# abignoli/EdgeGraph3D

Measured on AMD Instinct MI355X. Metric: triangulated edge-points/sec, higher is better.
Workload: dtype f64

## Files before the change

### edgegraph3d_amd/api.py

```python
import ctypes as C
import os

import numpy as np

from . import _cdefs as D

_LIB = None


class Eg3dError(RuntimeError):
    pass


def lib_path():
    return os.environ.get("EG3D_LIB") or os.path.join(os.path.dirname(os.path.abspath(__file__)), "libeg3d.so")


def lib():
    global _LIB
    if _LIB is None:
        path = lib_path()
        if not os.path.exists(path):
            raise Eg3dError("libeg3d.so (HIP extension) is missing: run `python -m edgegraph3d_amd.build`. "
                            "There is no CPU fallback.")
# ... 159 lines not shown
        return None
    return C.c_void_p(x.ptr if isinstance(x, DeviceArray) else int(x))


class Context:
    def __init__(self, scene_ptr, device=0, _handle=None):
        self._h = C.c_void_p()
        if _handle is not None:
            self._h = _handle
        else:
            _check(lib().eg3d_create(scene_ptr, device, C.byref(self._h)), "eg3d_create")
        nv, dv = C.c_int32(), C.c_int32()
        _check(lib().eg3d_context_info(self._h, C.byref(nv), C.byref(dv)), "eg3d_context_info")
        self.n_views, self.device = nv.value, dv.value

    def clone(self):
        h = C.c_void_p()
        _check(lib().eg3d_clone(self._h, C.byref(h)), "eg3d_clone")
        return Context(None, _handle=h)

    def set_pipelining(self, lanes=0, units=0):
        _check(lib().eg3d_set_pipelining(self._h, lanes, units), "eg3d_set_pipelining")

    def close(self):
        if self._h:
            lib().eg3d_destroy(self._h)
            self._h = C.c_void_p()

    def __del__(self):
        try:
            self.close()
        except Exception:
            pass

    def grid(self, view, which):
        ncols, nrows = C.c_uint32(), C.c_uint32()
        off, ids = D.u32p(), D.u32p()
        _check(lib().eg3d_get_grid(self._h, view, which, C.byref(ncols), C.byref(nrows), C.byref(off), C.byref(ids)),
               "eg3d_get_grid")
        n = ncols.value * nrows.value
        o = D.as_np(off, n + 1, np.uint32)
        return ncols.value, nrows.value, o, D.as_np(ids, int(o[-1]), np.uint32)

    def upload_seeds(self, seeds_ptr):
        _check(lib().eg3d_upload_seeds(self._h, seeds_ptr), "eg3d_upload_seeds")

# ... 308 lines not shown
```

### edgegraph3d_amd/csrc/eg3d_api.hip

```cpp
#include <hip/hip_runtime.h>
#include <hipcub/hipcub.hpp>

#include <algorithm>
#include <cstdio>
#include <cstdlib>

#include <atomic>
#include <chrono>
#include <cmath>
#include <cstring>
#include <memory>
#include <mutex>
#include <string>
#include <thread>
#include <vector>

#include "../../include/eg3d_host.h"
#include "eg3d_api_internal.h"
#include "eg3d_host_copy.h"

thread_local std::string eg3d::api::g_err;
extern "C" const char* eg3d_last_error(void) { return g_err.c_str(); }

static std::atomic<int64_t> g_live_device_bytes{0};
// ... 948 lines not shown
extern "C" int eg3d_probe_hyp_sections(eg3d_ctx* c, double* sum, double* slowest, uint32_t* counts) {
  if (!c || !sum || !slowest || !counts) return EG3D_ERR_ARG;
  const uint32_t n = c->last_nhyp;
  std::vector<HypResult> r(n ? n : 1);
  if (n) HIP_TRY(hipMemcpy(r.data(), c->b_res.p, sizeof(HypResult) * n, hipMemcpyDeviceToHost));
  for (int k = 0; k < 6; k++) sum[k] = slowest[k] = 0;
  for (int k = 0; k < 5; k++) counts[k] = 0;
  counts[0] = n;
  for (uint32_t h = 0; h < n; h++) {
    if (r[h].status & HYP_TRI) counts[1]++;
    if (r[h].status & HYP_D1) counts[2]++;
    if (r[h].status & HYP_D2) counts[3]++;
    if (hyp_compatible(r[h].status, r[h].n1, r[h].n2)) counts[4]++;
    sum[0] += r[h].n1;
    sum[1] += r[h].n2;
    if (r[h].n1 > slowest[0]) slowest[0] = r[h].n1;
    if (r[h].n2 > slowest[1]) slowest[1] = r[h].n2;
    if (r[h].n1 + r[h].n2 >= 32) sum[2] += 1;
  }
  return EG3D_OK;
}

#endif
#if defined(EG3D_WITH_K3C_ENGINE) && (defined(EG3D_SECTION_TIMING) || defined(EG3D_K3C_TIMING))
namespace eg3d { int k3c_dbg_read(unsigned long long* out, int reset); }
extern "C" int eg3d_probe_k3c(unsigned long long* out128, int reset) { return eg3d::k3c_dbg_read(out128, reset); }
#endif
```

### edgegraph3d_amd/csrc/eg3d_api_internal.h

```cpp
#pragma once
#include <hip/hip_runtime.h>

#include <algorithm>
#include <chrono>
#include <cstdlib>
#include <cstring>
#include <initializer_list>
#include <memory>
#include <mutex>
#include <string>
#include <vector>

#include "../../include/eg3d.h"
#include "eg3d_kernels.h"
#include "eg3d_k8_replay.h"
#include "eg3d_k9_polymatch.h"
#include "eg3d_k10_simgraph.h"
#include "eg3d_k11_louvain.h"

#define EG3D_API_BEGIN namespace eg3d { namespace api __attribute__((visibility("hidden"))) {
#define EG3D_API_END }}

EG3D_API_BEGIN
extern thread_local std::string g_err;
// ... 146 lines not shown

using namespace eg3d;
using namespace eg3d::api;

struct eg3d_ctx {
  int device = 0;
  Tunables tune;
  hipStream_t stream = nullptr;
  int V = 0, W = 0, H = 0;
  DevScene ds;
  DevBuf b_camP, b_F, b_Fv, b_vpo, b_pvo, b_vtx, b_pls, b_ple, b_g30o, b_g30i, b_g4o, b_g4i, b_bbo, b_bb;
  std::shared_ptr<DevOwner> scene_owner;
  std::shared_ptr<HostGrids> hg;
  uint32_t gw[2] = {0, 0}, gh[2] = {0, 0};
  uint32_t grid_dropped = 0;
  uint32_t n_seeds = 0;
  std::shared_ptr<std::vector<uint32_t>> h_trk;
  DevBuf b_toff, b_tview, b_txy;
  std::shared_ptr<DevOwner> seeds_owner;
  WorkBuf b_sv_seed, b_map_view, b_map_entry, b_map_n, b_raw_cnt, b_raw_off, b_cand_pl, b_start_hits, b_cand_cnt,
      b_start_cnt, b_task_off, b_task_seed, b_task_entry, b_task_hit, b_task_k, b_task_list_off, b_list_cnt, b_list_ptr,
      b_hits, b_tasks, b_nhyp, b_hyp_off, b_res, b_arena, b_ctr, b_cs_task, b_valid, b_chain_off, b_chains,
      b_cscratch, b_couts, b_cpts, b_cobs, b_cpoff, b_cooff, b_scan_tmp, b_scanchk, b_cost, b_cidx, b_cost2, b_order, b_redo[2];
  WorkBuf o_X, o_off, o_view, o_pl, o_seg, o_xy, o_key;
  WorkBuf f_X, f_off, f_view, f_xy, f_Xo, f_inl;
  WorkBuf r_hist, r_blk, r_Xo, r_inl, c_X, c_off, c_view, c_pl, c_seg, c_xy, c_key;
  bool compact_nt = false;
  WorkBuf d_first, d_cnt, d_keep;
  bool dedup_valid = false;
  WorkBuf prim_tmp;
  WorkBuf k8_cnt, k8_slot, k8_last, k8_firstof, k8_flag, k8_rank, k8_lastof, k8_plid, k8_key[2], k8_val[2], k8_map, k8_sflag, k8_pos;
  WorkBuf g_nodeX, g_nodept, g_pls, g_ple, g_conoff, g_conpl, g_ivoff, g_ivss, g_ivsxy, g_ives, g_ivexy;
  WorkBuf k9_svseed, k9_cnt, k9_pl, k9_dist, k9_acc, k9_accoff, k9_first, k9_parent, k9_root, k9_ckey, k9_rank, k9_key[2], k9_ctr,
      k9_ref, k9_rowoff, k9_plids;
  WorkBuf k10_svseed, k10_cnt, k10_off, k10_pair[2], k10_crkey, k10_cpoff, k10_cpview, k10_cppl, k10_croff, k10_crpoint, k10_weight, k10_vis,
      k10_npairs, k10_pairoff, k10_nkey[2], k10_nodeof, k10_nodeg, k10_nodeview, k10_nodepl, k10_edge[2], k10_dkey[2], k10_dval[2],
      k10_adjoff, k10_adjnode, k10_ctr;
  WorkBuf k11[K11B_COUNT];
  uint32_t louvain_log2_slots = 0;
  uint64_t simgraph_pair_budget = 0;
  int replay_table_bits = 0;
  uint32_t n_pl = 0, n_vtx = 0;
  WorkBuf b_sets_off, b_sets_ids;
  WorkBuf b_fscratch, b_queue, b_items;
  WorkBuf b_pools, b_stage_pts, b_stage_obs, b_stage_used;
  uint32_t slots_per_xcd = 0;
// ... 125 lines not shown
```

### edgegraph3d_amd/csrc/eg3d_api_match.hip

```cpp
#include <sys/mman.h>

#include <atomic>
#include <condition_variable>
#include <cstdio>
#include <shared_mutex>
#include <thread>

#include "eg3d_api_internal.h"
#include "eg3d_host_copy.h"

#ifndef EG3D_D2H_CHUNK
#define EG3D_D2H_CHUNK ((size_t)16 << 20)
#endif
#define EG3D_D2H_CHUNK_SMALL ((size_t)2 << 20)
#define EG3D_D2H_BIG_CLOUD ((size_t)96 << 20)
#ifndef EG3D_D2H_RING
#define EG3D_D2H_RING 4
#endif
static int ensure_d2h_ring(eg3d_ctx* c, size_t cloud_bytes) {
  const size_t want = cloud_bytes >= EG3D_D2H_BIG_CLOUD ? EG3D_D2H_CHUNK : EG3D_D2H_CHUNK_SMALL;
  if (c->pinned && c->ring_chunk >= want) return EG3D_OK;
  if (c->pinned) (void)hipHostFree(c->pinned);
  c->pinned = nullptr;
  c->ring_chunk = c->pinned_cap = 0;
// ... 339 lines not shown
    const int ic = rb.add(c->b_ctr.p, sizeof(Counters) / 4);
    const int it = rb.add(c->b_chain_off.as<uint32_t>() + nt, 1);
    const int iw = rb.add(c->b_scanchk.as<uint32_t>(), 1);
    rb.clear_after(c->b_scanchk.as<uint32_t>());
    BUF_TRY(rb.run());
    memcpy(&hc, rb.item(ic), sizeof(Counters));
    if (c->tune.trace_arena)
      fprintf(stderr, "eg3d: hypothesis arena: %u hypotheses, %u points used of %u (%.2f per hypothesis)%s\n", B.n_hyp,
              hc.arena_used, arena_cap, B.n_hyp ? (double)hc.arena_used / B.n_hyp : 0.0,
              (hc.flags & CTR_ARENA_OVERFLOW) ? " OVERFLOW" : "");
    if (!(hc.flags & CTR_ARENA_OVERFLOW)) {
      if (*rb.item(iw)) return wrapped_error("chains");
      B.n_chains = *rb.item(it);
      break;
    }
    if (attempt >= 6) {
      g_err = "eg3d: hypothesis arena overflow";
      return EG3D_ERR_CAPACITY;
    }
    arena_cap = std::max<uint32_t>(arena_cap * 2, hc.arena_used + (hc.arena_used >> 2));
    if (B.n_hyp) c->arena_per_hyp = std::max(c->arena_per_hyp, 1.25 * (double)arena_cap / (double)B.n_hyp);
  }
  H.flags |= (hc.flags & 0xffu);
  BUF_TRY(c->b_chains.ensure(sizeof(ChainSeed) * (B.n_chains + 1)));
  launch_compact_chains(st, nt, c->b_cs_task.as<ChainSeed>(), c->b_valid.as<uint32_t>(), c->b_chain_off.as<uint32_t>(),
                        c->b_chains.as<ChainSeed>());
  HIP_TRY(hipEventRecord(c->eb[4], st));
  return EG3D_OK;
}

struct ExpandState {
  uint32_t c0 = 0, nc = 0;
  uint32_t redo_n = 0;
  int redo_buf = 0;
  uint64_t stage_lim_pts = ~0ull, stage_lim_obs = ~0ull;
  ChainLayout L{};
  bool engine = false;
  uint32_t eng_waves = 0, eng_lanes = 64;
  SlotPools pools{};
  StageBuf stage{};
  uint32_t n_launch = 0;
  const uint32_t* launch_order = nullptr;
  Counters hc{};
  uint32_t np = 0, no = 0;
  unsigned long long stage_used[2] = {0, 0};
  float ms_expand = 0, ms_emit = 0;
// ... 1146 lines not shown
```

### edgegraph3d_amd/csrc/eg3d_dev_geom.h

```cpp
#pragma once
#include <stdint.h>

#if defined(__HIPCC__)
#include <hip/hip_runtime.h>
#define EG3D_HD __host__ __device__ inline
#define EG3D_HD_FLAT __host__ __device__ inline __attribute__((always_inline))
#else
#define EG3D_HD inline
#define EG3D_HD_FLAT inline
#endif

#if defined(__HIP_DEVICE_COMPILE__)
#define EG3D_SQRTF(x) __builtin_sqrtf(x)
#define EG3D_SQRT(x) __dsqrt_rn(x)
#else
#include <math.h>
#define EG3D_SQRTF(x) sqrtf(x)
#define EG3D_SQRT(x) sqrt(x)
#endif

#ifndef EG3D_STAT
#define EG3D_STAT(i)
#endif

// ... 397 lines not shown
        got = true;
        seg_found = (uint32_t)(to_start ? first - k : first + k - 1);
        break;
      }
      W.shift(k);
    }
    if (!got) return WALK_EXTREME;
  }
  out.seg = seg_found;
  out.x = hx;
  out.y = hy;
  if (bounded) {
    float dsq = dist2(hx, hy, p.x, p.y);
    if (dsq < (min_d * min_d) || dsq > (max_d * max_d)) return WALK_BOUND;
  }
  return WALK_FOUND;
}
template <class VPtr>
EG3D_HD uint32_t walk_by_line_pf(const PlRefT<VPtr>& pl, const PlPt& p, uint32_t direction, float la, float lb, float lc,
                                 bool bounded, float min_d, float max_d, PlPt& out) {
  VtxWindow<VPtr> W;
  if (!walk_by_line_open(pl, p, direction, W)) return WALK_BAD_DIR;
  return walk_by_line_run(pl, p, direction, la, lb, lc, bounded, min_d, max_d, W, out);
}

EG3D_HD float polyline_closest(const PlRef& pl, float px, float py, PlPt& out) {
  float bx, by;
  float best = seg_closest(px, py, pl.v[0].x, pl.v[0].y, pl.v[1].x, pl.v[1].y, bx, by);
  uint32_t bseg = 0;
  for (uint32_t i = 2; i < pl.n; i++) {
    float cx, cy;
    float d = seg_closest(px, py, pl.v[i - 1].x, pl.v[i - 1].y, pl.v[i].x, pl.v[i].y, cx, cy);
    if (d < best) {
      best = d;
      bx = cx;
      by = cy;
      bseg = i - 1;
    }
  }
  out.seg = bseg;
  out.x = bx;
  out.y = by;
  return best;
}

EG3D_HD float polyline_closest_range(const PlRef& pl, float px, float py, uint32_t s0, uint32_t s1, PlPt& out) {
// ... 155 lines not shown
```

### edgegraph3d_amd/csrc/eg3d_k3a_engine.h

```cpp
#pragma once
#include "eg3d_dev_pipeline.h"

#include "eg3d_dev_coopgn.h"

namespace eg3d {

#ifdef EG3D_GN_COUNTERS
#define K3A_T0() unsigned long long kt_[3] = {0, 0, 0}, kc_[4] = {0, 0, 0, 0}, kt0_ = __builtin_readcyclecounter(), kt1_
#define K3A_T(i) (kt1_ = __builtin_readcyclecounter(), kt_[i] += kt1_ - kt0_, kt0_ = kt1_)
#define K3A_C(i, v) (kc_[i] += (v))
#define K3A_TEND(kern)                                                \
  if (lane == 0) {                                                    \
    for (int q_ = 0; q_ < 3; q_++) EG3D_GN_DBG(113 + 7 * (kern) + q_, kt_[q_]); \
    for (int q_ = 0; q_ < 4; q_++) EG3D_GN_DBG(116 + 7 * (kern) + q_, kc_[q_]); \
  }
#else
#define K3A_T0() ((void)0)
#define K3A_T(i) ((void)0)
#define K3A_C(i, v) ((void)0)
#define K3A_TEND(kern) ((void)0)
#endif

#define EG3D_K3A_STAGE EG3D_K3A_STAGE_POINTS
#ifndef EG3D_K3A_SPEC
// ... 42 lines not shown
    return r;
  }
};

__device__ __forceinline__ uint32_t k3a_slots_per_lane(uint32_t n_working) {
  uint32_t k = 64u / n_working, p = 1;
  while (p * 2 <= k && p * 2 <= (uint32_t)EG3D_K3A_SPEC) p *= 2;
  return p;
}

__device__ __forceinline__ void k3a_serve(K3aShared& sh, const DevScene& s, uint32_t lane) {
  __syncthreads();
  if (sh.reqM[lane] & 1u) {
    const Obs o[3] = {sh.req[lane][0], sh.req[lane][1], sh.req[lane][2]};
    float X[3] = {0.0f, 0.0f, 0.0f};
    uint32_t f = 0;
    const bool ok = triangulate3(s.cam_P, o, X, f);
    sh.resX[lane][0] = X[0];
    sh.resX[lane][1] = X[1];
    sh.resX[lane][2] = X[2];
    sh.resF[lane] = (ok ? 1u : 0u) | (f << 8);
  }
  __syncthreads();
}

__device__ __forceinline__ HPoint k3a_point_of_slot(const K3aShared& sh, uint32_t slot) {
  HPoint hp;
  hp.X[0] = sh.resX[slot][0];
  hp.X[1] = sh.resX[slot][1];
  hp.X[2] = sh.resX[slot][2];
  hp.nobs = 3;
  hp.o[0] = sh.req[slot][0];
  hp.o[1] = sh.req[slot][1];
  hp.o[2] = sh.req[slot][2];
  hp.pad = 0;
  return hp;
}

enum : uint32_t { K3A_IDLE = 0, K3A_GEN = 1, K3A_REQ = 2, K3A_END = 3 };
enum : uint32_t { K3A_TRI0 = 0, K3A_ORIENT = 1, K3A_REPLAY = 2, K3A_OPP = 3 };

__global__ void __launch_bounds__(64, EG3D_K3A_WAVES) k3a_orient(DevScene s, StageAView a, const TaskDesc* tasks,
                                                                 const uint32_t* hyp_off, uint32_t n_hyp, HypResult* res,
                                                                 uint32_t cap, HPoint* arena, uint32_t arena_cap,
                                                                 Counters* ctr, uint32_t* queue, uint32_t lanes_per_wave,
                                                                 uint32_t* items, uint32_t* n_items) {
// ... 37 lines not shown
  auto issue = [&](uint32_t slot, int q, uint32_t round_off) {
    const PlPt pA = L.get(0), pB = L.get(1 + (q >> 1)), pC = L.get(3 + (q & 1));
    Obs o;
    o.view = (uint32_t)view[0];
    o.pl = pl[0];
    o.seg = pA.seg;
    o.x = pA.x;
    o.y = pA.y;
    sh.req[slot][0] = o;
    o.view = (uint32_t)view[1];
    o.pl = pl[1];
    o.seg = pB.seg;
    o.x = pB.x;
    o.y = pB.y;
    sh.req[slot][1] = o;
    o.view = (uint32_t)view[2];
    o.pl = pl[2];
    o.seg = pC.seg;
    o.x = pC.x;
    o.y = pC.y;
    sh.req[slot][2] = o;
    sh.reqM[slot] = 1u | ((uint32_t)q << 8) | (round_off << 10);
  };
  K3A_T0();

  for (;;) {
    const unsigned long long working = __ballot(!(st == K3A_IDLE && exhausted));
    if (!working) break;
    K3A_C(0, 1);
    K3A_C(2, __popcll(working));
    const uint32_t K = k3a_slots_per_lane((uint32_t)__popcll(working));
    const uint32_t slot0 = (uint32_t)__popcll(working & lt) * K;
    sh.reqM[lane] = 0;
    __syncthreads();
    uint32_t n_issued = 0;
    if (st == K3A_END) {
      bool finish = false, to_d1 = false, restart = false;
      if (phase == K3A_TRI0) {
        if (okmask & 1u) {
          status |= HYP_TRI;
          e = 0;
          phase = K3A_ORIENT;
          restart = true;
        } else {
          finish = true;
        }
// ... 96 lines not shown
        const TaskDesc d = tasks[t_cur];
        Obs c[3];
        hypothesis_hits(a, d, t_cur, h - hyp_off[t_cur], c);
        for (int k = 0; k < 3; k++) {
          view[k] = (int32_t)c[k].view;
          pl[k] = c[k].pl;
          L.load_polyline(s, k, view[k], pl[k]);
        }
        to_hits(c);
        status = 0;
        flags = 0;
        n1 = n2 = 0;
        base = 0xffffffffu;
        arena_ok = false;
        for (int k = 0; k < 3; k++) d1[k] = d2[k] = 0;
        X0[0] = X0[1] = X0[2] = 0.0f;
        phase = K3A_TRI0;
        reqmask = 1u;
        okmask = 0;
        st = K3A_REQ;
      }
    }
    dead_round = 0xffffffffu;
    if (st == K3A_GEN) {
      uint32_t walkers = alive;
      for (uint32_t round_off = 0;; round_off++) {
        uint32_t fl = 0, m = walkers;
        const PlRef pa = L.polyline(s, 0);
        PlPt q;
        const uint32_t w = walk_by_distance_pf(pa, L.get(0), dirA, EG3D_FOLLOW_STEP, q);
        if (w & WALK_BAD_DIR) fl |= 8u;
        if (w & WALK_EXTREME) {
          m = 0;
        } else {
          L.set(0, q);
          float la = 0.0f, lb = 0.0f, lc = 0.0f;
          PlRef pk = pa;
#pragma unroll 1
          for (int idx = 0; idx < 4 && m; idx++) {
            const int k = 1 + (idx >> 1), j = idx & 1;
            const uint32_t users = k == 1 ? (3u << (2 * j)) : (5u << j);
            if (j == 0) {
              if (!epiline(s.F, s.F_valid, s.n_views, view[0], view[k], q.x, q.y, la, lb, lc)) {
                m = 0;
                break;
              }
              pk = L.polyline(s, k);
            }
            if (!(m & users)) continue;
            PlPt r;
            const uint32_t wr = walk_by_line_pf(pk, L.get(2 * k - 1 + j), k == 1 ? dirB[j] : dirC[j], la, lb, lc, false, 0.0f,
                                                0.0f, r);
            if (wr & WALK_BAD_DIR) fl |= 8u;
            if (wr & WALK_FOUND)
              L.set(2 * k - 1 + j, r);
            else
              m &= ~users;
          }
        }
        if (phase != K3A_REPLAY) flags |= fl;
        if (round_off == 0) {
          reqmask = m;
          okmask = 0;
          if (!m) {
            if (phase == K3A_REPLAY) n1 = i_rep;
            if (phase == K3A_ORIENT) {
              alive = 0;
              rounds++;
            }
            st = K3A_END;
            break;
          }
          st = K3A_REQ;
          while (reqmask && n_issued < K) {
            const int qq = __ffs((int)reqmask) - 1;
            reqmask &= reqmask - 1u;
            issue(slot0 + n_issued, qq, 0u);
            n_issued++;
          }
          if (reqmask) break;
        } else {
          if (!m) {
            if (phase == K3A_REPLAY)
              n1 = i_rep + round_off;
            else
              dead_round = round_off;
            break;
          }
          uint32_t mm = m;
          while (mm) {
            const int qq = __ffs((int)mm) - 1;
            mm &= mm - 1u;
            issue(slot0 + n_issued, qq, round_off);
            n_issued++;
          }
        }
        const uint32_t cm = (uint32_t)__popc(m);
        bool more;
        if (phase == K3A_REPLAY)
          more = i_rep + round_off + 1u < n1 && n_issued < K;
        else if (phase == K3A_ORIENT)
          more = cm >= 2u && n_issued + cm <= K && round_off < 14u;
        else
          more = false;
        if (!more) break;
        walkers = m;
      }
    }
    if (st == K3A_REQ && n_issued == 0) {
      while (reqmask && n_issued < K) {
        const int qq = __ffs((int)reqmask) - 1;
        reqmask &= reqmask - 1u;
        issue(slot0 + n_issued, qq, 0u);
        n_issued++;
      }
    }
    K3A_T(0);
    K3A_C(1, __popcll(__ballot(sh.reqM[lane] & 1u)));
    k3a_serve(sh, s, lane);
    K3A_T(1);
    if (n_issued) {
      if (phase == K3A_REPLAY) {
        for (uint32_t j = 0; j < n_issued; j++)
          if (arena_ok) arena[base + i_rep + j] = k3a_point_of_slot(sh, slot0 + j);
        i_rep += n_issued;
        st = K3A_END;
      } else if (phase == K3A_ORIENT) {
        uint32_t cur = 0;
        bool decided = false;
// ... 28 lines not shown
          }
          st = K3A_END;
        }
      } else {
        const uint32_t f = sh.resF[slot0];
        flags |= f >> 8;
        if (f & 1u) {
          okmask |= 1u;
          if (phase == K3A_TRI0) {
            X0[0] = sh.resX[slot0][0];
            X0[1] = sh.resX[slot0][1];
            X0[2] = sh.resX[slot0][2];
          } else {
            status |= HYP_D2;
            n2 = 1;
            if (arena_ok) arena[base + n1] = k3a_point_of_slot(sh, slot0);
          }
        }
        st = K3A_END;
      }
    }
    K3A_T(2);
  }
  K3A_TEND(0);
}

template <class T>
__device__ __forceinline__ T k3a_pick(const T a[3], int i) {
  return i == 0 ? a[0] : i == 1 ? a[1] : a[2];
}
__device__ __forceinline__ bool k3a_follow_request(const DevScene& s, const K3aLane& L, const int32_t view3[3],
                                                   int st_start, const uint32_t dirs[3], const int32_t ids[3],
                                                   int& st_used, PlPt sel_pt[3], uint32_t& fl) {
#pragma unroll 1
  for (int st = st_start; st < 3; st++) {
    const int32_t sv = k3a_pick(view3, st);
    const int sd = (sv == ids[0]) ? 0 : (sv == ids[1]) ? 1 : 2;
    const PlRef ps = L.polyline(s, sd);
    PlPt q;
    const uint32_t w = walk_by_distance_pf(ps, L.get(3 + st), k3a_pick(dirs, sd), EG3D_FOLLOW_STEP, q);
    if (w & WALK_BAD_DIR) fl |= 8u;
    if (w & WALK_EXTREME) continue;
    int found = 0;
    PlPt r1 = q, r2 = q;
#pragma unroll 1
    for (int t = 0; t < 2; t++) {
      const int i = t == 0 ? (st == 0 ? 1 : 0) : (st == 2 ? 1 : 2);
      const int32_t cv = k3a_pick(view3, i);
      float la, lb, lc;
      if (!epiline(s.F, s.F_valid, s.n_views, sv, cv, q.x, q.y, la, lb, lc)) continue;
      const int cd = (cv == ids[0]) ? 0 : (cv == ids[1]) ? 1 : 2;
      const PlRef pk = L.polyline(s, cd);
      PlPt r;
      const uint32_t wr =
          walk_by_line_pf(pk, L.get(3 + i), k3a_pick(dirs, cd), la, lb, lc, true, EG3D_FOLLOW_MIN, EG3D_FOLLOW_MAX, r);
      if (wr & WALK_BAD_DIR) fl |= 8u;
      if (wr & WALK_FOUND) {
        found++;
        if (t == 0)
          r1 = r;
        else
          r2 = r;
      }
    }
    if (found < 2) continue;
    st_used = st;
    sel_pt[0] = q;
    sel_pt[1] = r1;
    sel_pt[2] = r2;
    return true;
  }
  return false;
}

__global__ void __launch_bounds__(64, EG3D_K3A_WAVES) k3a_follow_spec(DevScene s, HypResult* res, HPoint* scratch,
                                                                      uint32_t cap, HPoint* arena, uint32_t arena_cap,
                                                                      Counters* ctr, uint32_t* queue, uint32_t lanes_per_wave,
                                                                      const uint32_t* items, const uint32_t* n_items_p) {
  __shared__ K3aShared sh;
  const uint32_t lane = threadIdx.x;
  const K3aLane L{&sh, lane};
  const unsigned long long lt = (1ull << lane) - 1ull;
  const uint32_t stage = cap < (uint32_t)EG3D_K3A_STAGE ? cap : (uint32_t)EG3D_K3A_STAGE;
  HPoint* scr = scratch + ((size_t)blockIdx.x * 64 + lane) * stage;
  uint32_t big_base = 0xffffffffu;
  const uint32_t n_items = *n_items_p;
  bool have = false, exhausted = lane >= lanes_per_wave;
  uint32_t h = 0, dir = 0, n_init = 0, n_new = 0, init_off = 0, flags = 0;
  int st_start = 0;
  uint32_t dirs[3] = {0, 0, 0};
  int32_t ids[3] = {0, 0, 0};
  int32_t cview[3] = {0, 0, 0};
  uint32_t cpl[3] = {0, 0, 0};
  K3A_T0();
  for (;;) {
    while (!have && !exhausted) {
      const uint32_t i = atomicAdd(queue, 1u);
      if (i >= n_items) {
        exhausted = true;
        break;
      }
      const uint32_t item = items[i];
      h = item >> 1;
      dir = item & 1u;
      const HypResult& r = res[h];
      const uint32_t stt = r.status;
      if (!(dir == 0 ? (stt & HYP_D1) : (stt & HYP_D2))) continue;
      n_init = dir == 0 ? r.n1 : r.n2;
      init_off = dir == 0 ? r.pts1_off : r.pts2_off;
      if (n_init == 0 || init_off == 0xffffffffu) continue;
      for (int k = 0; k < 3; k++) dirs[k] = dir == 0 ? r.dirs1[k] : r.dirs2[k];
      const HPoint last = arena[init_off + n_init - 1];
      for (int k = 0; k < 3; k++) {
        cview[k] = (int32_t)last.o[k].view;
        cpl[k] = last.o[k].pl;
        ids[k] = cview[k];
        L.load_polyline(s, k, cview[k], cpl[k]);
        PlPt p;
        p.seg = last.o[k].seg;
        p.x = last.o[k].x;
        p.y = last.o[k].y;
        L.set(k, p);
      }
      n_new = 0;
      flags = 0;
      st_start = 0;
      big_base = 0xffffffffu;
      have = true;
    }
    const unsigned long long working = __ballot(have);
    if (!working) break;
    const uint32_t K = k3a_slots_per_lane((uint32_t)__popcll(working));
    const uint32_t slot0 = (uint32_t)__popcll(working & lt) * K;
    sh.reqM[lane] = 0;
    __syncthreads();
    uint32_t n_req = 0, end_fl = 0;
    bool ended = false;
    if (have) {
      const uint32_t total = n_init + n_new;
      const uint32_t room = total < cap ? cap - total : 0u;
      const uint32_t lim = K < room + 1u ? K : room + 1u;
      int32_t bview[3] = {cview[0], cview[1], cview[2]};
      uint32_t bpl[3] = {cpl[0], cpl[1], cpl[2]};
      L.set(3, L.get(0));
      L.set(4, L.get(1));
      L.set(5, L.get(2));
      int st0 = st_start;
      while (n_req < lim) {
        int st_used = 0;
        PlPt sel_pt[3];
        uint32_t fl = 0;
        if (!k3a_follow_request(s, L, bview, st0, dirs, ids, st_used, sel_pt, fl)) {
          ended = true;
          end_fl = fl;
          break;
        }
        const uint32_t slot = slot0 + n_req;
        int32_t nview[3];
        uint32_t npl[3];
        const int sel_idx[3] = {st_used, st_used == 0 ? 1 : 0, st_used == 2 ? 1 : 2};
        for (int k = 0; k < 3; k++) {
          nview[k] = k3a_pick(bview, sel_idx[k]);
          npl[k] = k3a_pick(bpl, sel_idx[k]);
          Obs o;
          o.view = (uint32_t)nview[k];
          o.pl = npl[k];
          o.seg = sel_pt[k].seg;
          o.x = sel_pt[k].x;
          o.y = sel_pt[k].y;
          sh.req[slot][k] = o;
        }
        sh.reqM[slot] = 1u | ((uint32_t)st_used << 8) | (fl << 16);
        n_req++;
        for (int k = 0; k < 3; k++) {
          bview[k] = nview[k];
          bpl[k] = npl[k];
          L.set(3 + k, sel_pt[k]);
        }
        st0 = 0;
      }
    }
    K3A_T(0);
    K3A_C(0, 1);
    K3A_C(2, __popcll(working));
    K3A_C(1, __popcll(__ballot(sh.reqM[lane] & 1u)));
    k3a_serve(sh, s, lane);
    K3A_T(1);
    if (have) {
      bool finish = false;
      uint32_t j = 0;
      for (; j < n_req; j++) {
        const uint32_t slot = slot0 + j;
        const uint32_t m = sh.reqM[slot], f = sh.resF[slot];
        flags |= (m >> 16) | (f >> 8);
        if (f & 1u) {
          if (n_init + n_new >= cap) {
            flags |= 4u;
            finish = true;
            break;
          }
          if (big_base != 0xffffffffu)
            arena[big_base + n_init + n_new] = k3a_point_of_slot(sh, slot);
// ... 48 lines not shown
          if (base + total <= arena_cap) {
            for (uint32_t k = 0; k < n_init; k++) arena[base + k] = arena[init_off + k];
            for (uint32_t k = 0; k < n_new; k++) arena[base + n_init + k] = scr[k];
            if (dir == 0) {
              res[h].pts1_off = base;
              res[h].n1 = total;
            } else {
              res[h].pts2_off = base;
              res[h].n2 = total;
            }
          } else {
            atomicOr(&ctr->flags, CTR_ARENA_OVERFLOW);
          }
        }
        if (flags) {
          atomicOr(&ctr->flags, flags);
          atomicOr(&res[h].flags, flags);
        }
        have = false;
      }
    }
    K3A_T(2);
  }
  K3A_TEND(1);
}

}
```

### edgegraph3d_amd/csrc/eg3d_kernels.h

```cpp
#pragma once
#include <hip/hip_runtime.h>
#include <stdint.h>

#include "eg3d_dev_pipeline.h"
#include "eg3d_matched_core.h"

namespace eg3d {

struct SeedsDev {
  const uint32_t* trk_off;
  const int32_t* trk_view;
  const float* trk_xy;
};

__device__ __forceinline__ void seed_obs_in_view(const SeedsDev& sd, uint32_t t0, uint32_t k, int32_t view, float& x,
                                                 float& y) {
  x = 0.f;
  y = 0.f;
  for (uint32_t i = 0; i < k; i++)
    if (sd.trk_view[t0 + i] == view) {
      x = sd.trk_xy[2 * (t0 + i)];
      y = sd.trk_xy[2 * (t0 + i) + 1];
    }
}

enum : uint32_t { CTR_ARENA_OVERFLOW = 0x100u, CTR_SLOT_STARVED = 0x200u ,
                  CTR_LONG_REFUSED = 0x400u ,
                  CTR_N1_NO_PROGRESS = 0x800u  };
typedef uint64_t eg3d_off_t;
struct Counters {
  uint32_t arena_used;
  uint32_t flags;
  unsigned long long bytes;
  uint32_t max_chain_ticks;
  uint32_t pad_;
  unsigned long long hits_used;
};
inline dim3 blocks_for(uint64_t n, uint32_t per_block) { return dim3((unsigned)((n + per_block - 1) / per_block)); }

struct PubArgs {
  const uint32_t* src[6];
  uint32_t words[6];
  uint32_t* clear[3];
  int n, n_clear;
};
enum { EG3D_MBOX_WORDS = 64 };
void launch_publish(hipStream_t st, const PubArgs& a, uint32_t* mbox_dev, uint32_t seq);
void launch_scan_check(hipStream_t st, const uint32_t* out, uint64_t n_plus_one, uint32_t* wrapped);

#define EG3D_K0_PL_BITS_HOST 19
void launch_k0_pairs(hipStream_t st, bool fill, DevScene s, uint32_t n_pl, float cell_dim, int map_w, int map_h, uint32_t* cnt,
                     const uint32_t* off, unsigned long long* keys, uint32_t* dropped);
void launch_k0_csr(hipStream_t st, const unsigned long long* keys, uint32_t n, uint32_t total_cells, uint32_t* off, uint32_t* ids);

void launch_seed_prep(hipStream_t st, SeedsDev sd, uint32_t seed_begin, uint32_t n_seeds, uint32_t sv_base,
                      uint32_t* sv_seed, int32_t* map_view, uint32_t* map_entry, uint32_t* map_n);
void launch_k1_count_raw(hipStream_t st, DevScene s, SeedsDev sd, uint32_t sv_base, uint32_t n_sv, const uint32_t* sv_seed,
                         uint32_t* raw_cnt);
void launch_k1(hipStream_t st, DevScene s, SeedsDev sd, uint32_t sv_base, uint32_t n_sv, const uint32_t* sv_seed,
// ... 128 lines not shown
```

Baseline: 47.28 million.

## Split epipolar line walks into per-lane head plus wave-cooperative tail search

Each lane tests the first few polyline segments of an epipolar-line walk on its own. Any walk still undecided is then served by the whole 64-lane wavefront, which tests 64 segments per pass and picks the first hit by ballot. This targets the divergence where one long serial walk stalls the rest of the wave. The generate and follow loops are restructured to stay wave-uniform so every lane can join the cooperative search, and walk counters are added with atomics at kernel end. The trade-offs are extra broadcasts and ballots on every walk, plus register pressure from the restructured loops.

```diff
diff --git a/edgegraph3d_amd/api.py b/edgegraph3d_amd/api.py
--- a/edgegraph3d_amd/api.py
+++ b/edgegraph3d_amd/api.py
@@ -205,6 +205,15 @@
     def set_pipelining(self, lanes=0, units=0):
         _check(lib().eg3d_set_pipelining(self._h, lanes, units), "eg3d_set_pipelining")
 
+    def probe_k3a_walks(self):
+        L = lib()
+        if not hasattr(L, "eg3d_probe_k3a_walks"):
+            raise Eg3dError("eg3d_probe_k3a_walks: not in this library (test-only builds carry it)")
+        L.eg3d_probe_k3a_walks.argtypes = [C.c_void_p, C.POINTER(C.c_ulonglong)]
+        out = (C.c_ulonglong * 2)()
+        _check(L.eg3d_probe_k3a_walks(self._h, out), "eg3d_probe_k3a_walks")
+        return int(out[0]), int(out[1])
+
     def close(self):
         if self._h:
             lib().eg3d_destroy(self._h)
diff --git a/edgegraph3d_amd/csrc/eg3d_api.hip b/edgegraph3d_amd/csrc/eg3d_api.hip
--- a/edgegraph3d_amd/csrc/eg3d_api.hip
+++ b/edgegraph3d_amd/csrc/eg3d_api.hip
@@ -994,6 +994,20 @@
 }
 
 #endif
+#if defined(EG3D_WITH_K3C_ENGINE) || defined(EG3D_SECTION_TIMING)
+extern "C" int eg3d_probe_k3a_walks(eg3d_ctx* c, unsigned long long* out2) {
+  if (!c || !out2) return EG3D_ERR_ARG;
+  out2[0] = out2[1] = 0;
+  std::vector<eg3d_ctx*> all = c->lanes;
+  if (all.empty()) all.push_back(c);
+  for (eg3d_ctx* l : all) {
+    out2[0] += l->k3a_walks_served;
+    out2[1] += l->k3a_walk_passes;
+    l->k3a_walks_served = l->k3a_walk_passes = 0;
+  }
+  return EG3D_OK;
+}
+#endif
 #if defined(EG3D_WITH_K3C_ENGINE) && (defined(EG3D_SECTION_TIMING) || defined(EG3D_K3C_TIMING))
 namespace eg3d { int k3c_dbg_read(unsigned long long* out, int reset); }
 extern "C" int eg3d_probe_k3c(unsigned long long* out128, int reset) { return eg3d::k3c_dbg_read(out128, reset); }
diff --git a/edgegraph3d_amd/csrc/eg3d_api_internal.h b/edgegraph3d_amd/csrc/eg3d_api_internal.h
--- a/edgegraph3d_amd/csrc/eg3d_api_internal.h
+++ b/edgegraph3d_amd/csrc/eg3d_api_internal.h
@@ -192,6 +192,7 @@
       b_start_cnt, b_task_off, b_task_seed, b_task_entry, b_task_hit, b_task_k, b_task_list_off, b_list_cnt, b_list_ptr,
       b_hits, b_tasks, b_nhyp, b_hyp_off, b_res, b_arena, b_ctr, b_cs_task, b_valid, b_chain_off, b_chains,
       b_cscratch, b_couts, b_cpts, b_cobs, b_cpoff, b_cooff, b_scan_tmp, b_scanchk, b_cost, b_cidx, b_cost2, b_order, b_redo[2];
+  unsigned long long k3a_walks_served = 0, k3a_walk_passes = 0;
   WorkBuf o_X, o_off, o_view, o_pl, o_seg, o_xy, o_key;
   WorkBuf f_X, f_off, f_view, f_xy, f_Xo, f_inl;
   WorkBuf r_hist, r_blk, r_Xo, r_inl, c_X, c_off, c_view, c_pl, c_seg, c_xy, c_key;
diff --git a/edgegraph3d_amd/csrc/eg3d_api_match.hip b/edgegraph3d_amd/csrc/eg3d_api_match.hip
--- a/edgegraph3d_amd/csrc/eg3d_api_match.hip
+++ b/edgegraph3d_amd/csrc/eg3d_api_match.hip
@@ -385,6 +385,8 @@
     if (B.n_hyp) c->arena_per_hyp = std::max(c->arena_per_hyp, 1.25 * (double)arena_cap / (double)B.n_hyp);
   }
   H.flags |= (hc.flags & 0xffu);
+  c->k3a_walks_served += hc.k3a_walks_served;
+  c->k3a_walk_passes += hc.k3a_walk_passes;
   BUF_TRY(c->b_chains.ensure(sizeof(ChainSeed) * (B.n_chains + 1)));
   launch_compact_chains(st, nt, c->b_cs_task.as<ChainSeed>(), c->b_valid.as<uint32_t>(), c->b_chain_off.as<uint32_t>(),
                         c->b_chains.as<ChainSeed>());
diff --git a/edgegraph3d_amd/csrc/eg3d_dev_geom.h b/edgegraph3d_amd/csrc/eg3d_dev_geom.h
--- a/edgegraph3d_amd/csrc/eg3d_dev_geom.h
+++ b/edgegraph3d_amd/csrc/eg3d_dev_geom.h
@@ -443,6 +443,71 @@
   VtxWindow<VPtr> W;
   if (!walk_by_line_open(pl, p, direction, W)) return WALK_BAD_DIR;
   return walk_by_line_run(pl, p, direction, la, lb, lc, bounded, min_d, max_d, W, out);
+}
+
+enum : uint32_t { WALK_UNDECIDED = 0u };
+#define EG3D_WALK_HEAD_MAX 4
+struct WalkCont {
+  int32_t next;
+  int32_t step;
+  int32_t left;
+};
+EG3D_HD uint32_t walk_resolve(uint32_t r, uint32_t seg, float hx, float hy, const PlPt& p, bool bounded, float min_d,
+                              float max_d, PlPt& out) {
+  if (r & 2u) return WALK_QUASIPARALLEL;
+  if (!(r & 1u)) return WALK_EXTREME;
+  out.seg = seg;
+  out.x = hx;
+  out.y = hy;
+  if (bounded) {
+    float dsq = dist2(hx, hy, p.x, p.y);
+    if (dsq < (min_d * min_d) || dsq > (max_d * max_d)) return WALK_BOUND;
+  }
+  return WALK_FOUND;
+}
+template <class VPtr>
+EG3D_HD uint32_t walk_seg_test(VPtr v, const WalkCont& c, int32_t k, float la, float lb, float lc, const LineDir& ld,
+                               uint32_t& seg, float& hx, float& hy) {
+  const int32_t i0 = c.next + c.step * k, i1 = i0 + c.step;
+  seg = (uint32_t)(i0 < i1 ? i0 : i1);
+  const f2 a = v[i0], b = v[i1];
+  return seg_line_hit_guarded(a.x, a.y, b.x, b.y, la, lb, lc, ld, hx, hy);
+}
+template <int T, class VPtr>
+EG3D_HD uint32_t walk_by_line_head(const PlRefT<VPtr>& pl, const PlPt& p, uint32_t direction, float la, float lb, float lc,
+                                   const LineDir& ld, bool bounded, float min_d, float max_d, PlPt& out, WalkCont& c) {
+  static_assert(T >= 1 && T <= EG3D_WALK_HEAD_MAX, "the head tests what the window holds");
+  VtxWindow<VPtr> W;
+  if (!walk_by_line_open(pl, p, direction, W)) return WALK_BAD_DIR;
+  const int32_t count = W.stepv < 0 ? W.first + 1 : (int32_t)pl.n - W.first;
+  float hx = 0.0f, hy = 0.0f;
+  uint32_t seg = p.seg;
+  uint32_t r = seg_line_hit_guarded(p.x, p.y, W.w0.x, W.w0.y, la, lb, lc, ld, hx, hy);
+  int32_t k = 1;
+  if (!r && k < count) {
+    r = seg_line_hit_guarded(W.w0.x, W.w0.y, W.w1.x, W.w1.y, la, lb, lc, ld, hx, hy);
+    k = 2;
+    if (T >= 2 && !r && k < count) {
+      r = seg_line_hit_guarded(W.w1.x, W.w1.y, W.w2.x, W.w2.y, la, lb, lc, ld, hx, hy);
+      k = 3;
+      if (T >= 3 && !r && k < count) {
+        r = seg_line_hit_guarded(W.w2.x, W.w2.y, W.w3.x, W.w3.y, la, lb, lc, ld, hx, hy);
+        k = 4;
+        if (T >= 4 && !r && k < count) {
+          r = seg_line_hit_guarded(W.w3.x, W.w3.y, W.w4.x, W.w4.y, la, lb, lc, ld, hx, hy);
+          k = 5;
+        }
+      }
+    }
+    if (r) seg = (uint32_t)(W.stepv < 0 ? W.first - (k - 1) : W.first + (k - 1) - 1);
+  }
+  if (!r && k < count) {
+    c.next = W.first + W.stepv * (k - 1);
+    c.step = W.stepv;
+    c.left = count - k;
+    return WALK_UNDECIDED;
+  }
+  return walk_resolve(r, seg, hx, hy, p, bounded, min_d, max_d, out);
 }
 
 EG3D_HD float polyline_closest(const PlRef& pl, float px, float py, PlPt& out) {
diff --git a/edgegraph3d_amd/csrc/eg3d_k3a_engine.h b/edgegraph3d_amd/csrc/eg3d_k3a_engine.h
--- a/edgegraph3d_amd/csrc/eg3d_k3a_engine.h
+++ b/edgegraph3d_amd/csrc/eg3d_k3a_engine.h
@@ -88,6 +88,65 @@
     sh.resF[lane] = (ok ? 1u : 0u) | (f << 8);
   }
   __syncthreads();
+}
+
+#ifndef EG3D_K3A_WALK_HEAD
+#define EG3D_K3A_WALK_HEAD 4
+#endif
+struct K3aWalkStats {
+  uint32_t served = 0, passes = 0;
+};
+__device__ __forceinline__ uint32_t k3a_walk_coop(const DevScene& s, uint32_t lane, bool want, const PlRef& pl, const PlPt& p,
+                                                  uint32_t direction, float la, float lb, float lc, bool bounded, float min_d,
+                                                  float max_d, PlPt& out, K3aWalkStats& ws) {
+  uint32_t status = WALK_EXTREME;
+  WalkCont c;
+  c.next = c.left = 0;
+  c.step = 1;
+  LineDir ld;
+  ld.bx = ld.by = ld.bb = 0.0f;
+  bool pending = false;
+  if (want) {
+    ld = line_dir(la, lb);
+    status = walk_by_line_head<EG3D_K3A_WALK_HEAD>(pl, p, direction, la, lb, lc, ld, bounded, min_d, max_d, out, c);
+    pending = status == WALK_UNDECIDED;
+  }
+  unsigned long long pend = __ballot(pending);
+  while (pend) {
+    const int o = __ffsll((long long)pend) - 1;
+    pend &= pend - 1ull;
+    WalkCont oc;
+    oc.next = lane_bcast(c.next, o);
+    oc.step = lane_bcast(c.step, o);
+    oc.left = lane_bcast(c.left, o);
+    const f2* ov = s.vtx + lane_bcast((uint32_t)(pl.v - s.vtx), o);
+    const float ola = lane_bcast(la, o), olb = lane_bcast(lb, o), olc = lane_bcast(lc, o);
+    LineDir old;
+    old.bx = lane_bcast(ld.bx, o);
+    old.by = lane_bcast(ld.by, o);
+    old.bb = lane_bcast(ld.bb, o);
+    uint32_t rf = 0, sf = 0;
+    float xf = 0.0f, yf = 0.0f;
+    for (int32_t k0 = 0; k0 < oc.left; k0 += 64) {
+      ws.passes++;
+      const int32_t k = k0 + (int32_t)lane;
+      uint32_t r = 0, seg = 0;
+      float hx = 0.0f, hy = 0.0f;
+      if (k < oc.left) r = walk_seg_test(ov, oc, k, ola, olb, olc, old, seg, hx, hy);
+      const unsigned long long any = __ballot(r != 0);
+      if (any) {
+        const int f = __ffsll((long long)any) - 1;
+        rf = lane_bcast(r, f);
+        sf = lane_bcast(seg, f);
+        xf = lane_bcast(hx, f);
+        yf = lane_bcast(hy, f);
+        break;
+      }
+    }
+    ws.served++;
+    if (lane == (uint32_t)o) status = walk_resolve(rf, sf, xf, yf, p, bounded, min_d, max_d, out);
+  }
+  return status;
 }
 
 __device__ __forceinline__ HPoint k3a_point_of_slot(const K3aShared& sh, uint32_t slot) {
@@ -171,6 +230,7 @@
     sh.req[slot][2] = o;
     sh.reqM[slot] = 1u | ((uint32_t)q << 8) | (round_off << 10);
   };
+  K3aWalkStats wstat;
   K3A_T0();
 
   for (;;) {
@@ -313,35 +373,34 @@
       }
     }
     dead_round = 0xffffffffu;
-    if (st == K3A_GEN) {
-      uint32_t walkers = alive;
-      for (uint32_t round_off = 0;; round_off++) {
-        uint32_t fl = 0, m = walkers;
-        const PlRef pa = L.polyline(s, 0);
-        PlPt q;
-        const uint32_t w = walk_by_distance_pf(pa, L.get(0), dirA, EG3D_FOLLOW_STEP, q);
+    bool gen = st == K3A_GEN;
+    uint32_t walkers = alive;
+    for (uint32_t round_off = 0; __ballot(gen); round_off++) {
+      uint32_t fl = 0, m = gen ? walkers : 0u;
+      PlPt q;
+      q.seg = 0;
+      q.x = q.y = 0.0f;
+      if (gen) {
+        const uint32_t w = walk_by_distance_pf(L.polyline(s, 0), L.get(0), dirA, EG3D_FOLLOW_STEP, q);
         if (w & WALK_BAD_DIR) fl |= 8u;
-        if (w & WALK_EXTREME) {
+        if (w & WALK_EXTREME)
           m = 0;
-        } else {
+        else
           L.set(0, q);
-          float la = 0.0f, lb = 0.0f, lc = 0.0f;
-          PlRef pk = pa;
+      }
 #pragma unroll 1
-          for (int idx = 0; idx < 4 && m; idx++) {
-            const int k = 1 + (idx >> 1), j = idx & 1;
-            const uint32_t users = k == 1 ? (3u << (2 * j)) : (5u << j);
-            if (j == 0) {
-              if (!epiline(s.F, s.F_valid, s.n_views, view[0], view[k], q.x, q.y, la, lb, lc)) {
-                m = 0;
-                break;
-              }
-              pk = L.polyline(s, k);
-            }
-            if (!(m & users)) continue;
-            PlPt r;
-            const uint32_t wr = walk_by_line_pf(pk, L.get(2 * k - 1 + j), k == 1 ? dirB[j] : dirC[j], la, lb, lc, false, 0.0f,
-                                                0.0f, r);
+      for (int k = 1; k <= 2; k++) {
+        float la = 0.0f, lb = 0.0f, lc = 0.0f;
+        if (m && !epiline(s.F, s.F_valid, s.n_views, view[0], view[k], q.x, q.y, la, lb, lc)) m = 0;
+        const PlRef pk = L.polyline(s, k);
+#pragma unroll 1
+        for (int j = 0; j < 2; j++) {
+          const uint32_t users = k == 1 ? (3u << (2 * j)) : (5u << j);
+          const bool want = (m & users) != 0;
+          PlPt r;
+          const uint32_t wr = k3a_walk_coop(s, lane, want, pk, L.get(2 * k - 1 + j), k == 1 ? dirB[j] : dirC[j], la, lb, lc,
+                                            false, 0.0f, 0.0f, r, wstat);
+          if (want) {
             if (wr & WALK_BAD_DIR) fl |= 8u;
             if (wr & WALK_FOUND)
               L.set(2 * k - 1 + j, r);
@@ -349,53 +408,59 @@
               m &= ~users;
           }
         }
-        if (phase != K3A_REPLAY) flags |= fl;
-        if (round_off == 0) {
-          reqmask = m;
-          okmask = 0;
-          if (!m) {
-            if (phase == K3A_REPLAY) n1 = i_rep;
-            if (phase == K3A_ORIENT) {
-              alive = 0;
-              rounds++;
+      }
+      if (gen) {
+        bool more = false;
+        do {
+          if (phase != K3A_REPLAY) flags |= fl;
+          if (round_off == 0) {
+            reqmask = m;
+            okmask = 0;
+            if (!m) {
+              if (phase == K3A_REPLAY) n1 = i_rep;
+              if (phase == K3A_ORIENT) {
+                alive = 0;
+                rounds++;
+              }
+              st = K3A_END;
+              break;
             }
-            st = K3A_END;
-            break;
-          }
-          st = K3A_REQ;
-          while (reqmask && n_issued < K) {
-            const int qq = __ffs((int)reqmask) - 1;
-            reqmask &= reqmask - 1u;
-            issue(slot0 + n_issued, qq, 0u);
-            n_issued++;
-          }
-          if (reqmask) break;
-        } else {
-          if (!m) {
-            if (phase == K3A_REPLAY)
-              n1 = i_rep + round_off;
-            else
-              dead_round = round_off;
-            break;
-          }
-          uint32_t mm = m;
-          while (mm) {
-            const int qq = __ffs((int)mm) - 1;
-            mm &= mm - 1u;
-            issue(slot0 + n_issued, qq, round_off);
-            n_issued++;
-          }
-        }
-        const uint32_t cm = (uint32_t)__popc(m);
-        bool more;
-        if (phase == K3A_REPLAY)
-          more = i_rep + round_off + 1u < n1 && n_issued < K;
-        else if (phase == K3A_ORIENT)
-          more = cm >= 2u && n_issued + cm <= K && round_off < 14u;
+            st = K3A_REQ;
+            while (reqmask && n_issued < K) {
+              const int qq = __ffs((int)reqmask) - 1;
+              reqmask &= reqmask - 1u;
+              issue(slot0 + n_issued, qq, 0u);
+              n_issued++;
+            }
+            if (reqmask) break;
+          } else {
+            if (!m) {
+              if (phase == K3A_REPLAY)
+                n1 = i_rep + round_off;
+              else
+                dead_round = round_off;
+              break;
+            }
+            uint32_t mm = m;
+            while (mm) {
+              const int qq = __ffs((int)mm) - 1;
+              mm &= mm - 1u;
+              issue(slot0 + n_issued, qq, round_off);
+              n_issued++;
+            }
+          }
+          const uint32_t cm = (uint32_t)__popc(m);
+          if (phase == K3A_REPLAY)
+            more = i_rep + round_off + 1u < n1 && n_issued < K;
+          else if (phase == K3A_ORIENT)
+            more = cm >= 2u && n_issued + cm <= K && round_off < 14u;
+          else
+            more = false;
+        } while (false);
+        if (more)
+          walkers = m;
         else
-          more = false;
-        if (!more) break;
-        walkers = m;
+          gen = false;
       }
     }
     if (st == K3A_REQ && n_issued == 0) {
@@ -470,6 +535,10 @@
     }
     K3A_T(2);
   }
+  if (lane == 0 && wstat.served) {
+    atomicAdd(&ctr->k3a_walks_served, wstat.served);
+    atomicAdd(&ctr->k3a_walk_passes, wstat.passes);
+  }
   K3A_TEND(0);
 }
 
@@ -477,50 +546,6 @@
 __device__ __forceinline__ T k3a_pick(const T a[3], int i) {
   return i == 0 ? a[0] : i == 1 ? a[1] : a[2];
 }
-__device__ __forceinline__ bool k3a_follow_request(const DevScene& s, const K3aLane& L, const int32_t view3[3],
-                                                   int st_start, const uint32_t dirs[3], const int32_t ids[3],
-                                                   int& st_used, PlPt sel_pt[3], uint32_t& fl) {
-#pragma unroll 1
-  for (int st = st_start; st < 3; st++) {
-    const int32_t sv = k3a_pick(view3, st);
-    const int sd = (sv == ids[0]) ? 0 : (sv == ids[1]) ? 1 : 2;
-    const PlRef ps = L.polyline(s, sd);
-    PlPt q;
-    const uint32_t w = walk_by_distance_pf(ps, L.get(3 + st), k3a_pick(dirs, sd), EG3D_FOLLOW_STEP, q);
-    if (w & WALK_BAD_DIR) fl |= 8u;
-    if (w & WALK_EXTREME) continue;
-    int found = 0;
-    PlPt r1 = q, r2 = q;
-#pragma unroll 1
-    for (int t = 0; t < 2; t++) {
-      const int i = t == 0 ? (st == 0 ? 1 : 0) : (st == 2 ? 1 : 2);
-      const int32_t cv = k3a_pick(view3, i);
-      float la, lb, lc;
-      if (!epiline(s.F, s.F_valid, s.n_views, sv, cv, q.x, q.y, la, lb, lc)) continue;
-      const int cd = (cv == ids[0]) ? 0 : (cv == ids[1]) ? 1 : 2;
-      const PlRef pk = L.polyline(s, cd);
-      PlPt r;
-      const uint32_t wr =
-          walk_by_line_pf(pk, L.get(3 + i), k3a_pick(dirs, cd), la, lb, lc, true, EG3D_FOLLOW_MIN, EG3D_FOLLOW_MAX, r);
-      if (wr & WALK_BAD_DIR) fl |= 8u;
-      if (wr & WALK_FOUND) {
-        found++;
-        if (t == 0)
-          r1 = r;
-        else
-          r2 = r;
-      }
-    }
-    if (found < 2) continue;
-    st_used = st;
-    sel_pt[0] = q;
-    sel_pt[1] = r1;
-    sel_pt[2] = r2;
-    return true;
-  }
-  return false;
-}
-
 __global__ void __launch_bounds__(64, EG3D_K3A_WAVES) k3a_follow_spec(DevScene s, HypResult* res, HPoint* scratch,
                                                                       uint32_t cap, HPoint* arena, uint32_t arena_cap,
                                                                       Counters* ctr, uint32_t* queue, uint32_t lanes_per_wave,
@@ -540,6 +565,7 @@
   int32_t ids[3] = {0, 0, 0};
   int32_t cview[3] = {0, 0, 0};
   uint32_t cpl[3] = {0, 0, 0};
+  K3aWalkStats wstat;
   K3A_T0();
   for (;;) {
     while (!have && !exhausted) {
@@ -584,48 +610,92 @@
     __syncthreads();
     uint32_t n_req = 0, end_fl = 0;
     bool ended = false;
+    uint32_t lim = 0, fl = 0;
+    int32_t bview[3] = {cview[0], cview[1], cview[2]};
+    uint32_t bpl[3] = {cpl[0], cpl[1], cpl[2]};
+    int st = st_start;
     if (have) {
       const uint32_t total = n_init + n_new;
       const uint32_t room = total < cap ? cap - total : 0u;
-      const uint32_t lim = K < room + 1u ? K : room + 1u;
-      int32_t bview[3] = {cview[0], cview[1], cview[2]};
-      uint32_t bpl[3] = {cpl[0], cpl[1], cpl[2]};
+      lim = K < room + 1u ? K : room + 1u;
       L.set(3, L.get(0));
       L.set(4, L.get(1));
       L.set(5, L.get(2));
-      int st0 = st_start;
-      while (n_req < lim) {
-        int st_used = 0;
-        PlPt sel_pt[3];
-        uint32_t fl = 0;
-        if (!k3a_follow_request(s, L, bview, st0, dirs, ids, st_used, sel_pt, fl)) {
+    }
+    bool act = have;
+    if (act && st >= 3) {
+      ended = true;
+      act = false;
+    }
+    while (__ballot(act)) {
+      bool go = false;
+      int32_t sv = 0;
+      PlPt q;
+      q.seg = 0;
+      q.x = q.y = 0.0f;
+      if (act) {
+        sv = k3a_pick(bview, st);
+        const int sd = (sv == ids[0]) ? 0 : (sv == ids[1]) ? 1 : 2;
+        const uint32_t w = walk_by_distance_pf(L.polyline(s, sd), L.get(3 + st), k3a_pick(dirs, sd), EG3D_FOLLOW_STEP, q);
+        if (w & WALK_BAD_DIR) fl |= 8u;
+        go = !(w & WALK_EXTREME);
+      }
+      int found = 0;
+      PlPt r1 = q, r2 = q;
+#pragma unroll 1
+      for (int t = 0; t < 2; t++) {
+        const int i = t == 0 ? (st == 0 ? 1 : 0) : (st == 2 ? 1 : 2);
+        const int32_t cv = k3a_pick(bview, i);
+        float la = 0.0f, lb = 0.0f, lc = 0.0f;
+        const bool want = go && epiline(s.F, s.F_valid, s.n_views, sv, cv, q.x, q.y, la, lb, lc);
+        const int cd = (cv == ids[0]) ? 0 : (cv == ids[1]) ? 1 : 2;
+        PlPt r;
+        const uint32_t wr = k3a_walk_coop(s, lane, want, L.polyline(s, cd), L.get(3 + i), k3a_pick(dirs, cd), la, lb, lc, true,
+                                          EG3D_FOLLOW_MIN, EG3D_FOLLOW_MAX, r, wstat);
+        if (want) {
+          if (wr & WALK_BAD_DIR) fl |= 8u;
+          if (wr & WALK_FOUND) {
+            found++;
+            if (t == 0)
+              r1 = r;
+            else
+              r2 = r;
+          }
+        }
+      }
+      if (act) {
+        if (found == 2) {
+          const uint32_t slot = slot0 + n_req;
+          int32_t nview[3];
+          uint32_t npl[3];
+          const int sel_idx[3] = {st, st == 0 ? 1 : 0, st == 2 ? 1 : 2};
+          const PlPt sel_pt[3] = {q, r1, r2};
+          for (int k = 0; k < 3; k++) {
+            nview[k] = k3a_pick(bview, sel_idx[k]);
+            npl[k] = k3a_pick(bpl, sel_idx[k]);
+            Obs o;
+            o.view = (uint32_t)nview[k];
+            o.pl = npl[k];
+            o.seg = sel_pt[k].seg;
+            o.x = sel_pt[k].x;
+            o.y = sel_pt[k].y;
+            sh.req[slot][k] = o;
+          }
+          sh.reqM[slot] = 1u | ((uint32_t)st << 8) | (fl << 16);
+          n_req++;
+          for (int k = 0; k < 3; k++) {
+            bview[k] = nview[k];
+            bpl[k] = npl[k];
+            L.set(3 + k, sel_pt[k]);
+          }
+          st = 0;
+          fl = 0;
+          if (n_req >= lim) act = false;
+        } else if (++st >= 3) {
           ended = true;
           end_fl = fl;
-          break;
-        }
-        const uint32_t slot = slot0 + n_req;
-        int32_t nview[3];
-        uint32_t npl[3];
-        const int sel_idx[3] = {st_used, st_used == 0 ? 1 : 0, st_used == 2 ? 1 : 2};
-        for (int k = 0; k < 3; k++) {
-          nview[k] = k3a_pick(bview, sel_idx[k]);
-          npl[k] = k3a_pick(bpl, sel_idx[k]);
-          Obs o;
-          o.view = (uint32_t)nview[k];
-          o.pl = npl[k];
-          o.seg = sel_pt[k].seg;
-          o.x = sel_pt[k].x;
-          o.y = sel_pt[k].y;
-          sh.req[slot][k] = o;
-        }
-        sh.reqM[slot] = 1u | ((uint32_t)st_used << 8) | (fl << 16);
-        n_req++;
-        for (int k = 0; k < 3; k++) {
-          bview[k] = nview[k];
-          bpl[k] = npl[k];
-          L.set(3 + k, sel_pt[k]);
-        }
-        st0 = 0;
+          act = false;
+        }
       }
     }
     K3A_T(0);
@@ -720,6 +790,10 @@
     }
     K3A_T(2);
   }
+  if (lane == 0 && wstat.served) {
+    atomicAdd(&ctr->k3a_walks_served, wstat.served);
+    atomicAdd(&ctr->k3a_walk_passes, wstat.passes);
+  }
   K3A_TEND(1);
 }
 
diff --git a/edgegraph3d_amd/csrc/eg3d_kernels.h b/edgegraph3d_amd/csrc/eg3d_kernels.h
--- a/edgegraph3d_amd/csrc/eg3d_kernels.h
+++ b/edgegraph3d_amd/csrc/eg3d_kernels.h
@@ -35,6 +35,8 @@
   uint32_t max_chain_ticks;
   uint32_t pad_;
   unsigned long long hits_used;
+  uint32_t k3a_walks_served;
+  uint32_t k3a_walk_passes;
 };
 inline dim3 blocks_for(uint64_t n, uint32_t per_block) { return dim3((unsigned)((n + per_block - 1) / per_block)); }
 
```

Measured after the change: 48.25 million, median of 6. 2.1% higher.
